# spacejam/loghisto

Hardware: NVIDIA H100
Metric: histogram ingest throughput (samples/s) (higher is better)
Workload: dtype f64

## Files before the change

### loghisto_b200/csrc/lh_api.cu

```cuda
#include "../../include/loghisto_b200.h"
#include "lh_kernels.cuh"

#include <algorithm>
#include <cmath>
#include <condition_variable>
#include <cstdio>
#include <cstring>
#include <mutex>
#include <new>
#include <string>
#include <thread>
#include <vector>
#include <unistd.h>

using namespace lh;

namespace {

struct WriterEvent { cudaStream_t stream; cudaEvent_t ev; };

struct Scope { uint64_t ticket; int buf; cudaStream_t stream; std::thread::id thread; };
static_assert(sizeof(Prec) == sizeof(((lh_recorder *)0)->prec) && offsetof(lh_recorder, prec) % alignof(Prec) == 0,
              "lh_recorder.prec must hold an lh::Prec");

// ... 113 lines not shown
    uint32_t H = 0, C = 0;
    Prec pc{};
    Buffer buf[2];
    int active = 0;
    bool frozen = false;
    bool freezing = false;
    bool nnz_valid = false;
    cudaStream_t ingest_stream = nullptr, snap_stream = nullptr, copy_stream = nullptr;
    double *d_decomp = nullptr;
    unsigned long long *d_dropped = nullptr;
    double *d_ps[3] = {nullptr, nullptr, nullptr};
    char *d_res[3] = {nullptr, nullptr, nullptr};
    char *h_res[3] = {nullptr, nullptr, nullptr};
    cudaEvent_t res_done[3] = {nullptr, nullptr, nullptr};
    uint32_t res_np[3] = {0, 0, 0};
    uint64_t res_ticket[2] = {0, 0};
    uint64_t next_ticket = 1;
    uint32_t *d_nnz = nullptr, *d_offsets = nullptr;
    short *d_x_keys = nullptr; unsigned long long *d_x_counts = nullptr; size_t x_cap = 0;
    uint32_t *h_offsets = nullptr;
    short *h_x_keys = nullptr; unsigned long long *h_x_counts = nullptr; size_t hx_cap = 0;
    unsigned long long *h_counter_deltas = nullptr;
    std::vector<Slot> slots;
    uint64_t slot_seq = 0;
    size_t staging_bytes = 0;
    unsigned long long last_margin[2] = {0, 0};
    int k1_variant = kDefaultK1Variant;
    int k1_grid_mult = 1;
    int k1_reserve_sms = 0;
    int keyed_blocks_per_sm = 8;
    uint32_t hot_replicas = 1;
    int keyed_mode = 0;
    int64_t kp_chunk = 256 << 20;
    uint32_t wc_pf_tiles = 1;
    uint32_t wc_flush_samples = 24576;
    int wc_spt = 6;
    unsigned short *d_kp_queues = nullptr;
    unsigned int *d_kp_cnt = nullptr;
    uint4 *d_kp_rare = nullptr;
    size_t kp_cap = 0;
    int kp_parts = 0;
    const char *keyed_kernel = "";
    uint32_t comm_rank = 0, comm_world = 0;
    unsigned long long *d_comm = nullptr;
    unsigned int *d_comm_aux = nullptr;
    PeerMap peers[kMaxRanks];
    unsigned long long *d_red_buckets = nullptr;
    uint32_t *d_red_flags = nullptr;
    unsigned long long *d_red_counters = nullptr;
    bool view_reduced = false;
    bool view_counters_reduced = false;
    uint64_t comm_seq = 0;
    bool comm_two_shot = false;
    static constexpr int kCommRing = 8;
    cudaEvent_t comm_t0[kCommRing] = {}, comm_t1[kCommRing] = {};
    uint64_t ctx_id = 0;
    std::mutex rs_mu;
    cudaStream_t rs_stream = nullptr;
    unsigned long long *d_rs_rows = nullptr;
    uint32_t *d_rs_flags = nullptr, *d_rs_nnz = nullptr;
    bool rs_dirty = false;
    K1Variant k1[kNumK1Variants];
    static constexpr int kTimingRing = 16;
    cudaEvent_t ev_t0s[kTimingRing] = {}, ev_t1s[kTimingRing] = {};
    cudaEvent_t ev_t0 = nullptr, ev_t1 = nullptr;
    uint64_t ingest_seq = 0;
    bool timing_valid = false;
// ... 97 lines not shown
    const size_t cells = (size_t)ctx->H * 2u * ctx->pc.win;
    int grid = (int)std::min<size_t>((cells + 255) / 256, (size_t)ctx->sm_count * 16);
    k_fold_hot<<<grid, 256, 0, s>>>(ctx->buf[b].d_hot, ctx->buf[b].d_buckets, ctx->buf[b].d_flags, cells, ctx->hot_replicas, ctx->pc.win);
    LH_CUDA(ctx, cudaGetLastError());
    ctx->stats.kernel_launches++;
    ctx->buf[b].hot_pending = 0;
    return LH_OK;
}

KeyedOut keyed_out(lh_ctx *ctx, int b) {
    KeyedOut o{};
    o.hot = ctx->buf[b].d_hot; o.buckets = ctx->buf[b].d_buckets; o.flags = ctx->buf[b].d_flags;
    o.dropped = ctx->d_dropped; o.H = ctx->H;
    return o;
}

uint32_t ks_passes(const lh_ctx *ctx) {
    const uint32_t per_max = std::max<uint32_t>(1, (uint32_t)(KS_SMEM_BYTES / ((size_t)ctx->pc.win * 4)));
    return (ctx->H + per_max - 1) / per_max;
}

constexpr uint32_t KS_MAX_PASSES = 4;
bool small_route(const lh_ctx *ctx) { return ks_passes(ctx) <= KS_MAX_PASSES && ctx->keyed_mode == 0; }

template <typename IdT, typename ValT>
void launch_keyed_scalar(lh_ctx *ctx, const KeyedOut &ko, const IdT *ids, const ValT *vals, size_t n, cudaStream_t s) {
    if (!n) return;
    constexpr int T = 256;
    k_ingest_keyed<IdT, ValT, T><<<grid_1d(ctx, n, T, 1, ctx->keyed_blocks_per_sm), T, 0, s>>>(ids, vals, n, ko, ctx->pc);
    ctx->stats.kernel_launches++;
}

constexpr size_t kSmemBudget = 227 * 1024;
template <typename IdT, typename ValT, int SPT>
lh_status launch_keyed_wc_spt(lh_ctx *ctx, int b, const IdT *ids, const ValT *vals, size_t n4x4, cudaStream_t s, bool *used, size_t *taken,
                              const IdT *ids2 = nullptr, const long long *vals2 = nullptr, size_t n2 = 0, size_t *taken2 = nullptr) {
    *used = false;
    *taken = 0;
    if (taken2) *taken2 = 0;
    const int P = std::min(ctx->sm_count - ctx->k1_reserve_sms, (int)WC_MAX_PARTS);
    if (P < 8 || n4x4 + n2 == 0) return LH_OK;
    const uint32_t ids_per = (ctx->H + P - 1) / P;
    using S = WcShape<SPT>;
    const size_t hist_bytes = (((size_t)ids_per * ctx->pc.win + 3) & ~(size_t)3) * 4;
    uint32_t row_cap = 0;
    size_t smem = 0;
    for (uint32_t cap_try : {256u, 192u, 128u}) {
        smem = hist_bytes + 2 * WC_MAX_PARTS * 4 + (size_t)(P + 1) * (cap_try + WC_ROW_EXTRA) * 2;
        if (smem <= kSmemBudget) { row_cap = cap_try; break; }
    }
    if (!row_cap || (size_t)ids_per * ctx->pc.win > 65535) return LH_OK;
    if (ctx->keyed_mode != 2 && n4x4 + n2 < ((size_t)1 << 22)) return LH_OK;
    n4x4 = n4x4 / S::TILE * S::TILE;
    n2 = n2 / S::TILE * S::TILE;
    if (n4x4 + n2 == 0) return LH_OK;
    const size_t slice_max = std::max<size_t>(1, ((size_t)ctx->kp_chunk + (size_t)P * S::TILE - 1) / ((size_t)P * S::TILE));
    const size_t tiles_all = n4x4 / S::TILE + n2 / S::TILE;
    const size_t nchunks = (tiles_all + slice_max * P - 1) / (slice_max * P);
    const size_t slice_tiles = std::max<size_t>(1, (tiles_all + nchunks * P - 1) / (nchunks * P));
    const size_t expect = slice_max * S::TILE / P;
    const size_t cap = ((expect * 5 / 4 + 3 * WC_LINE + WC_LINE - 1) / WC_LINE) * WC_LINE;
    if (!ctx->d_kp_queues || ctx->kp_cap != cap || ctx->kp_parts != P) {
        cudaFree(ctx->d_kp_queues); cudaFree(ctx->d_kp_cnt); cudaFree(ctx->d_kp_rare);
        ctx->d_kp_queues = nullptr; ctx->d_kp_cnt = nullptr; ctx->d_kp_rare = nullptr;
        LH_CUDA(ctx, cudaMalloc(&ctx->d_kp_rare, (size_t)P * WC_RARE_CAP * sizeof(uint4)));
        LH_CUDA(ctx, cudaMalloc(&ctx->d_kp_queues, (size_t)2 * P * P * cap * sizeof(unsigned short)));
        LH_CUDA(ctx, cudaMalloc(&ctx->d_kp_cnt, ((size_t)2 * P * P + 1) * sizeof(unsigned int)));
        ctx->kp_cap = cap; ctx->kp_parts = P;
    }
    const void *fn = (const void *)k_ingest_keyed_wc<IdT, ValT, SPT, false>;
    if constexpr (std::is_same<ValT, double>::value) {
        if (n2) fn = (const void *)k_ingest_keyed_wc<IdT, double, SPT, true>;
    }
    LH_CUDA(ctx, cudaFuncSetAttribute(fn, cudaFuncAttributeMaxDynamicSharedMemorySize, (int)smem));
    unsigned int *d_barrier = ctx->d_kp_cnt + (size_t)2 * P * P;
    LH_CUDA(ctx, cudaMemsetAsync(d_barrier, 0, sizeof(unsigned int), s));
    WcParams prm{};
    prm.ids = ids; prm.vals = vals; prm.n = n4x4; prm.ids_per = ids_per; prm.cap = (uint32_t)cap;
    prm.ids2 = ids2; prm.vals2 = vals2; prm.n2 = n2;
    prm.inv_p = (uint32_t)(((uint64_t)1 << 32) / (uint64_t)P) + 1u;
    const double room = (double)row_cap - 63.0;
    const double m_max = std::pow((-3.5 + std::sqrt(3.5 * 3.5 + 4.0 * room)) / 2.0, 2.0);
    const uint32_t flush_samples = std::min<uint32_t>(ctx->wc_flush_samples, (uint32_t)(m_max * P));
    prm.flush_tiles = std::max<uint32_t>(1u, flush_samples / S::TILE);
    prm.pf_tiles = ctx->wc_pf_tiles;
    prm.row_cap = row_cap;
    prm.row_stride = row_cap + WC_ROW_EXTRA;
    prm.slice_tiles = (uint32_t)slice_tiles; prm.queues = ctx->d_kp_queues; prm.q_cnt = ctx->d_kp_cnt;
    prm.barrier = d_barrier; prm.rare = ctx->d_kp_rare; prm.o = keyed_out(ctx, b);
    Prec pc = ctx->pc;
    void *args[] = {&prm, &pc};
    LH_CUDA(ctx, cudaLaunchCooperativeKernel(fn, dim3(P), dim3(S::THREADS), args, smem, s));
    ctx->stats.kernel_launches++;
    *used = true;
    *taken = n4x4;
    if (taken2) *taken2 = n2;
    return LH_OK;
}
template <typename IdT, typename ValT>
lh_status launch_keyed_wc(lh_ctx *ctx, int b, const IdT *ids, const ValT *vals, size_t n4x4, cudaStream_t s, bool *used, size_t *taken,
                          const IdT *ids2 = nullptr, const long long *vals2 = nullptr, size_t n2 = 0, size_t *taken2 = nullptr) {
#define LH_WC_SHAPE(code) case code: return launch_keyed_wc_spt<IdT, ValT, code>(ctx, b, ids, vals, n4x4, s, used, taken, ids2, vals2, n2, taken2);
    switch (ctx->wc_spt) {
        LH_WC_SHAPE(6) LH_WC_SHAPE(4) LH_WC_SHAPE(3)
        default: return launch_keyed_wc_spt<IdT, ValT, 8>(ctx, b, ids, vals, n4x4, s, used, taken, ids2, vals2, n2, taken2);
    }
#undef LH_WC_SHAPE
}

template <typename IdT, typename ValT>
lh_status launch_keyed(lh_ctx *ctx, int b, const IdT *d_ids, const ValT *d_vals, size_t n, cudaStream_t s) {
    constexpr int T = 256;
    const KeyedOut ko = keyed_out(ctx, b);
    size_t done = 0;
    while (done < n) {
        const unsigned long long kCap = 0xFFFFFFFFull;
        if (ctx->buf[b].hot_pending >= kCap - (1ull << 30)) { lh_status st = fold_hot(ctx, b, s); if (st != LH_OK) return st; }
        size_t m = (size_t)std::min<unsigned long long>(n - done, kCap - ctx->buf[b].hot_pending);
        const IdT *ids = d_ids + done;
        const ValT *vals = d_vals + done;
        size_t head = std::min<size_t>(m, ((32u - ((uintptr_t)vals & 31u)) & 31u) / 8u);
        bool vec_ok = (((uintptr_t)(ids + head)) & (4 * sizeof(IdT) - 1)) == 0;
        size_t n4 = vec_ok ? (m - head) / 4 : 0;
        size_t tail_off = head + n4 * 4;
        if (!vec_ok) { head = 0; tail_off = 0; }
        launch_keyed_scalar(ctx, ko, ids, vals, head, s);
// ... 1294 lines not shown
    LH_ENTER(ctx);
    LH_CUDA(ctx, cudaMemcpy(d_dst, h_src, bytes, cudaMemcpyHostToDevice));
    return LH_OK;
}
extern "C" lh_status lh_memcpy_d2h(lh_ctx *ctx, void *h_dst, const void *d_src, size_t bytes) {
    LH_ENTER(ctx);
    LH_CUDA(ctx, cudaMemcpy(h_dst, d_src, bytes, cudaMemcpyDeviceToHost));
    return LH_OK;
}

extern "C" lh_status lh_tune(lh_ctx *ctx, const char *key, int64_t value) {
    LH_ENTER(ctx);
    if (!key) return fail(ctx, LH_ERR_INVALID, "key is NULL");
    if (!strcmp(key, "k1")) {
        if (value < 0 || value >= kNumK1Variants) return fail(ctx, LH_ERR_RANGE, "unknown k1 variant");
        ctx->k1_variant = (int)value;
        return LH_OK;
    }
    if (!strcmp(key, "k1_grid_mult")) {
        if (value < 1 || value > 64) return fail(ctx, LH_ERR_RANGE, "k1_grid_mult out of range");
        ctx->k1_grid_mult = (int)value;
        return LH_OK;
    }
    if (!strcmp(key, "k1_reserve_sms")) {
        if (value < 0 || value >= ctx->sm_count) return fail(ctx, LH_ERR_RANGE, "k1_reserve_sms out of range");
        ctx->k1_reserve_sms = (int)value;
        return LH_OK;
    }
    if (!strcmp(key, "keyed_mode")) {
        if (value < 0 || value > 2) return fail(ctx, LH_ERR_RANGE, "keyed_mode is 0 (auto), 1 (L2 atomics) or 2 (owner-partitioned, write-combining)");
        ctx->keyed_mode = (int)value;
        return LH_OK;
    }
    if (!strcmp(key, "wc_pf")) {
        if (value < 0 || value > 8) return fail(ctx, LH_ERR_RANGE, "wc_pf is 0 ... 8 tiles");
        ctx->wc_pf_tiles = (uint32_t)value;
        return LH_OK;
    }
    if (!strcmp(key, "wc_flush")) {
        if (value < 4096 || value > 65536) return fail(ctx, LH_ERR_RANGE, "wc_flush is 4096 ... 65536 samples");
        ctx->wc_flush_samples = (uint32_t)value;
        return LH_OK;
    }
    if (!strcmp(key, "wc_spt")) {
        if (value != 4 && value != 6 && value != 3 && value != 8)
            return fail(ctx, LH_ERR_RANGE, "wc_spt is a shape code: 6 (896 threads x 4 samples), 4 (1024 x 4), 3 (768 x 4) or 8 (512 x 8)");
        ctx->wc_spt = (int)value;
        return LH_OK;
    }
    if (!strcmp(key, "kp_chunk")) {
        if (value < (1 << 16) || value > ((int64_t)1 << 28)) return fail(ctx, LH_ERR_RANGE, "kp_chunk out of range");
        ctx->kp_chunk = value;
        return LH_OK;
    }
    if (!strcmp(key, "keyed_blocks_per_sm")) {
        if (value < 1 || value > 32) return fail(ctx, LH_ERR_RANGE, "keyed_blocks_per_sm out of range");
        ctx->keyed_blocks_per_sm = (int)value;
        return LH_OK;
    }
    return fail(ctx, LH_ERR_INVALID, "unknown tuning key");
}

extern "C" int32_t lh_k1_variant_count(void) { return kNumK1Variants; }
extern "C" int32_t lh_k1_variant_current(lh_ctx *ctx) { return ctx ? ctx->k1_variant : -1; }
extern "C" const char *lh_k1_variant_name(lh_ctx *ctx, int32_t i) {
    if (!ctx || i < 0 || i >= kNumK1Variants) return "";
    return ctx->k1[i].name;
}

extern "C" uint64_t lh_ingest_seq(lh_ctx *ctx) {
    if (!ctx) return 0;
// ... 24 lines not shown
```

### loghisto_b200/csrc/lh_kernels.cuh

```cuda
#pragma once
#include "../../include/loghisto_b200.h"
#include <type_traits>
#include "lh_device.cuh"

namespace lh {

struct f64x4 { double a, b, c, d; };
__device__ __forceinline__ uint64_t policy_evict_first() {
    uint64_t p;
    asm("createpolicy.fractional.L2::evict_first.b64 %0, 1.0;" : "=l"(p));
    return p;
}
__device__ __forceinline__ void ldg_stream_u64x4(const void *p, unsigned long long (&r)[4]) {
    const uint64_t pol = policy_evict_first();
    asm volatile("ld.global.nc.L1::no_allocate.L2::cache_hint.v2.b64 {%0, %1}, [%2], %3;"
                 : "=l"(r[0]), "=l"(r[1]) : "l"(p), "l"(pol));
    asm volatile("ld.global.nc.L1::no_allocate.L2::cache_hint.v2.b64 {%0, %1}, [%2], %3;"
                 : "=l"(r[2]), "=l"(r[3]) : "l"((const char *)p + 16), "l"(pol));
}
__device__ __forceinline__ f64x4 ldg_stream_f64x4(const void *p) {
    unsigned long long u[4];
    ldg_stream_u64x4(p, u);
    f64x4 r;
    r.a = __longlong_as_double((long long)u[0]); r.b = __longlong_as_double((long long)u[1]);
// ... 415 lines not shown
        if (__any_sync(0xFFFFFFFFu, any)) {
#pragma unroll
            for (int i = 0; i < 4; i++) {
                if (!flag[i]) continue;
                ValT rv;
                memcpy(&rv, &cur[i], 8);
                keyed_one<ValT>(cur_id[i], rv, pc, o, o.hot, pol);
                off[i] = trash_off;
            }
        }
#pragma unroll
        for (int i = 0; i < 4; i++) atomicAdd(reinterpret_cast<uint32_t *>(reinterpret_cast<char *>(ks_hist) + off[i]), 1u);
#pragma unroll
        for (int i = 0; i < 4; i++) { cur[i] = nxt[i]; cur_id[i] = nxt_id[i]; }
    }
    __syncthreads();
    for (uint32_t i = threadIdx.x; i < words; i += KS_THREADS) {
        const uint32_t c = ks_hist[i];
        if (!c) continue;
        const uint32_t lid = i / row, slot = i - lid * row;
        atomicAdd(&o.hot[(size_t)(id_lo + lid) * (2u * pc.win) + slot], c);
    }
}

constexpr int WC_MAX_PARTS = 160;
constexpr int WC_LINE = 64;

template <int SPT> struct WcShape {
    static constexpr int THREADS = SPT == 4 ? 1024 : SPT == 6 ? 896 : SPT == 3 ? 768 : 512;
    static constexpr int PER = SPT == 8 ? 8 : 4;
    static constexpr int TILE = THREADS * PER;
};
constexpr int WC_ROW_EXTRA = WC_LINE + 8;

struct WcParams {
    const void *ids;
    const void *vals;
    size_t n;
    const void *ids2;
    const void *vals2;
    size_t n2;
    uint32_t ids_per;
    uint32_t cap;
    uint32_t slice_tiles;
    uint32_t inv_p;
    uint32_t flush_tiles;
    uint32_t pf_tiles;
    uint32_t row_cap;
    uint32_t row_stride;
    unsigned short *queues;
    unsigned int *q_cnt;
    unsigned int *barrier;
    uint4 *rare;
    KeyedOut o;
};
constexpr uint32_t WC_RARE_CAP = 8192;

__device__ __forceinline__ void grid_barrier(unsigned int *bar, unsigned int target) {
    __syncthreads();
    if (threadIdx.x == 0) {
        __threadfence();
        atomicAdd(bar, 1u);
        unsigned int v;
        do {
            asm volatile("ld.acquire.gpu.global.u32 %0, [%1];" : "=r"(v) : "l"(bar) : "memory");
        } while (v < target);
    }
    __syncthreads();
}

__device__ __forceinline__ void wc_spill(uint32_t rec, uint32_t owner, uint32_t P, const Prec &pc, const KeyedOut &o) {
    const uint32_t lid = rec / pc.win, slot = rec - lid * pc.win, id = lid * P + owner;
    add_bucket_global(o.buckets + (size_t)id * 65536u, o.flags + id, slot, 1ull, pc.win);
}

template <typename IdT, typename ValT, int SPT, bool PAIR = false>
__global__ void __launch_bounds__(WcShape<SPT>::THREADS, 1)
k_ingest_keyed_wc(WcParams prm, Prec pc) {
    static_assert(!PAIR || std::is_same<ValT, double>::value, "the int64 segment rides on the float64 instantiation");
    using S = WcShape<SPT>;
    constexpr int WC_THREADS = S::THREADS;
    constexpr int GROUPS = S::PER / 4;
    extern __shared__ __align__(16) unsigned char wc_smem[];
    const uint32_t P = gridDim.x, p = blockIdx.x, tid = threadIdx.x;
    unsigned int *s_hist = reinterpret_cast<unsigned int *>(wc_smem);
    const uint32_t hist_words = prm.ids_per * pc.win;
    unsigned int *s_fill = s_hist + ((hist_words + 3u) & ~3u);
    unsigned int *s_off = s_fill + WC_MAX_PARTS;
    unsigned short *s_buf = reinterpret_cast<unsigned short *>(s_off + WC_MAX_PARTS);
    uint32_t fill_addr = smem_u32(s_fill);
    const uint32_t hist_addr = smem_u32(s_hist);
    asm volatile("mov.b32 %0, %0;" : "+r"(fill_addr));
    const uint32_t buf_addr = fill_addr + 2u * WC_MAX_PARTS * 4u;
    unsigned int *s_rare = s_fill + (WC_MAX_PARTS - 1);
    uint4 *rareq = prm.rare + (size_t)p * WC_RARE_CAP;
    uint32_t negP = 0u - P;
    asm volatile("mov.b32 %0, %0;" : "+r"(negP));

    for (uint32_t i = tid; i < hist_words; i += WC_THREADS) s_hist[i] = 0;
    if (tid < WC_MAX_PARTS) { s_fill[tid] = 0; s_off[tid] = 0; }
    uint32_t one_bits;
    asm volatile("mov.b32 %0, 0x3F800000;" : "=r"(one_bits));
    __syncthreads();

    const size_t tiles_seg0 = prm.n / S::TILE;
    const size_t tiles_total = tiles_seg0 + (PAIR ? prm.n2 / S::TILE : 0);
    const size_t chunk_tiles = (size_t)prm.slice_tiles * P;
    const size_t nchunks = (tiles_total + chunk_tiles - 1) / chunk_tiles;
    const IdT *ids = reinterpret_cast<const IdT *>(prm.ids);
    const unsigned int cap = prm.cap;
    const uint32_t row_cap = prm.row_cap, row_stride = prm.row_stride;


    unsigned long long cur[GROUPS][4], nxt[GROUPS][4];
    IdPack<IdT> cur_id[GROUPS], nxt_id[GROUPS];
    uint32_t since_flush = 0;
    const char *vptr = nullptr;
    const IdT *iptr = nullptr;
    const size_t pf_v = (size_t)prm.pf_tiles * S::TILE * 8, pf_i = (size_t)prm.pf_tiles * S::TILE;
    auto load_tile = [&](const char *vp, const IdT *ip, unsigned long long (&raw)[GROUPS][4], IdPack<IdT> (&idp)[GROUPS]) {
#pragma unroll
        for (int g = 0; g < GROUPS; g++) {
            load_vals4(vp, (size_t)g * WC_THREADS, raw[g]);
            idp[g].load(ip, (size_t)g * WC_THREADS);
        }
    };

    for (size_t c = 0; c < nchunks; c++) {
        const size_t par = c & 1;
        unsigned short *qset = prm.queues + par * (size_t)P * P * cap;
        unsigned int *cset = prm.q_cnt + par * (size_t)P * P;
        const bool last_chunk = c + 1 == nchunks;
        const size_t tile0 = c * chunk_tiles + (size_t)p * prm.slice_tiles;
        const uint32_t ntile_all = tile0 >= tiles_total ? 0u : (uint32_t)min((size_t)prm.slice_tiles, tiles_total - tile0);
        auto bin_tile = [&](unsigned long long (&raw)[GROUPS][4], IdPack<IdT> (&idp)[GROUPS], const bool as_i64) {
            if constexpr (PAIR) {
                if (as_i64) {
#pragma unroll
                    for (int g = 0; g < GROUPS; g++)
#pragma unroll
                        for (int j = 0; j < 4; j++) raw[g][j] = (unsigned long long)__double_as_longlong(__ll2double_rn((long long)raw[g][j]));
                }
            }
#pragma unroll
            for (int g = 0; g < GROUPS; g++) {
                double v[4];
#pragma unroll
                for (int j = 0; j < 4; j++) { ValT r; memcpy(&r, &raw[g][j], 8); v[j] = sample_to_f64<ValT>(r); }
                uint32_t idx[4];
                bool flag[4];
                bucket_offsets_v2<4, false, 0>(v, pc, one_bits, idx, flag);
                bool any = false;
#pragma unroll
                for (int j = 0; j < 4; j++) {
                    const uint32_t id = idp[g].get(j);
                    const uint32_t lid = __umulhi(id, prm.inv_p), owner = lid * negP + id;
                    const uint32_t rec = lid * pc.win + idx[j];
                    const bool rare = flag[j] | (id >= prm.o.H);
                    const uint32_t oe = rare ? P : owner;
                    uint32_t pos;
                    asm volatile("atom.shared.add.u32 %0, [%1], 1;" : "=r"(pos) : "r"(fill_addr + oe * 4u) : "memory");
                    flag[j] = rare | (pos >= row_cap);
                    if (!flag[j])
                        asm volatile("st.shared.u16 [%0], %1;" ::"r"(buf_addr + (oe * row_stride + pos) * 2u), "h"((unsigned short)rec) : "memory");
                    any |= flag[j];
                }
                if (__any_sync(0xFFFFFFFFu, any)) {
#pragma unroll
                    for (int j = 0; j < 4; j++)
                        if (flag[j]) {
                            const unsigned int at = atomicAdd(s_rare, 1u);
                            if (at < WC_RARE_CAP) rareq[at] = make_uint4((unsigned int)raw[g][j], (unsigned int)(raw[g][j] >> 32), idp[g].get(j), 0u);
                            else keyed_one_slow<ValT>(idp[g].get(j), raw[g][j], pc, prm.o);
                        }
                }
            }
            if (++since_flush == prm.flush_tiles) {
                since_flush = 0;
                __syncthreads();
                constexpr uint32_t GROUPS_PER_WARP = 8;
                const uint32_t sub = (tid & 31) >> 2, k4 = (tid & 3) * 2;
                for (uint32_t base = (tid >> 5) * GROUPS_PER_WARP; base < P; base += (WC_THREADS / 32) * GROUPS_PER_WARP) {
                    const uint32_t o = base + sub;
                    const bool act = o < P;
                    unsigned int n = 0, nfull = 0, off0 = 0;
                    uint4 keep0 = make_uint4(0, 0, 0, 0), keep1 = keep0;
                    uint4 *src = reinterpret_cast<uint4 *>(s_buf + (act ? o : 0) * row_stride);
                    if (act) {
                        n = min(s_fill[o], row_cap);
                        nfull = n / WC_LINE;
                        off0 = s_off[o];
                        unsigned short *qbase = qset + ((size_t)o * P + p) * cap;
                        keep0 = src[nfull * 8 + k4];
                        keep1 = src[nfull * 8 + k4 + 1];
                        for (unsigned int l = 0; l < nfull; l++) {
                            if (off0 + WC_LINE <= cap) {
                                uint4 *dst = reinterpret_cast<uint4 *>(qbase + off0);
                                const uint4 a0 = src[l * 8 + k4], a1 = src[l * 8 + k4 + 1];
                                dst[k4] = a0;
                                dst[k4 + 1] = a1;
                                off0 += WC_LINE;
                            } else if (k4 == 0) {
                                const unsigned short *r = s_buf + o * row_stride + l * WC_LINE;
                                for (unsigned int k = 0; k < (unsigned int)WC_LINE; k++) wc_spill(r[k], o, P, pc, prm.o);
                            }
                        }
                    }
                    __syncwarp();
                    if (act) {
                        if (nfull) { src[k4] = keep0; src[k4 + 1] = keep1; }
                        if (k4 == 0) { s_off[o] = off0; s_fill[o] = n - nfull * WC_LINE; }
                    }
                }
                __syncthreads();
            }
        };
        for (int part = 0; part < (PAIR ? 2 : 1); part++) {
            const size_t lo = part == 0 ? tile0 : max(tile0, tiles_seg0);
            const size_t hi = part == 0 ? min(tile0 + ntile_all, tiles_seg0) : tile0 + ntile_all;
            if (hi <= lo) continue;
            const uint32_t ntile = (uint32_t)(hi - lo);
            const bool as_i64 = part == 1;
            const size_t first = (part == 0 ? lo : lo - tiles_seg0) * S::TILE + (size_t)tid * 4;
            vptr = reinterpret_cast<const char *>(part == 0 ? prm.vals : prm.vals2) + first * 8;
            iptr = (part == 0 ? ids : reinterpret_cast<const IdT *>(prm.ids2)) + first;
            load_tile(vptr, iptr, cur, cur_id);
            auto prefetch_ahead = [&](uint32_t tile_loaded) {
                if (prm.pf_tiles && tile_loaded + prm.pf_tiles < ntile) {
#pragma unroll
                    for (int g = 0; g < GROUPS; g++) {
                        asm volatile("prefetch.global.L2 [%0];" ::"l"(vptr + pf_v + (size_t)g * WC_THREADS * 32));
                        if ((tid & 3) == 0) asm volatile("prefetch.global.L2 [%0];" ::"l"(iptr + pf_i + (size_t)g * WC_THREADS * 4));
                    }
                }
            };
            for (uint32_t t = 0; t < ntile; t += 2) {
                vptr += (size_t)S::TILE * 8;
                iptr += S::TILE;
                if (t + 1 < ntile) load_tile(vptr, iptr, nxt, nxt_id);
                prefetch_ahead(t + 1);
                bin_tile(cur, cur_id, as_i64);
                if (t + 1 >= ntile) break;
                vptr += (size_t)S::TILE * 8;
                iptr += S::TILE;
                if (t + 2 < ntile) load_tile(vptr, iptr, cur, cur_id);
                prefetch_ahead(t + 2);
                bin_tile(nxt, nxt_id, as_i64);
            }
        }
        __syncthreads();
        {
            const unsigned int nr = min(*s_rare, WC_RARE_CAP);
            for (unsigned int i = tid; i < nr; i += WC_THREADS) {
                const uint4 e = rareq[i];
                ValT r;
                const unsigned long long raw = ((unsigned long long)e.y << 32) | e.x;
                memcpy(&r, &raw, 8);
                keyed_one_direct<ValT>(e.z, r, pc, prm.o);
            }
            __syncthreads();
            if (tid == 0) *s_rare = 0;
        }
        if (last_chunk) {
            if (tid < P) {
                const uint32_t o = tid;
                const unsigned int n = min(s_fill[o], row_cap);
                unsigned int off0 = s_off[o];
                const uint4 *src = reinterpret_cast<const uint4 *>(s_buf + o * row_stride);
                for (unsigned int l = 0; l * WC_LINE < n; l++) {
                    const unsigned int nrec = min((unsigned int)WC_LINE, n - l * WC_LINE);
                    if (off0 + WC_LINE <= cap) {
                        uint4 *dst = reinterpret_cast<uint4 *>(qset + ((size_t)o * P + p) * cap + off0);
#pragma unroll
                        for (int k = 0; k < 8; k++) dst[k] = src[l * 8 + k];
                        off0 += nrec;
                    } else {
                        const unsigned short *r = s_buf + o * row_stride + l * WC_LINE;
                        for (unsigned int k = 0; k < nrec; k++) wc_spill(r[k], o, P, pc, prm.o);
                    }
                }
                s_off[o] = off0;
                s_fill[o] = 0;
            }
            __syncthreads();
        }
        if (tid < P) { cset[(size_t)tid * P + p] = s_off[tid]; }
        grid_barrier(prm.barrier, (unsigned int)((c + 1) * (size_t)P));
        if (tid < P) s_off[tid] = __ldcg(&cset[(size_t)p * P + tid]);
        __syncthreads();
        {
            const unsigned short *qmine = qset + (size_t)p * P * cap;
            const uint32_t lane = tid & 31;
#define LH_WC_INC2(word)                                                                                              \
            asm volatile("red.shared.add.u32 [%0], 1;" ::"r"(hist_addr + (((word) << 2) & 0x3FFFCu)) : "memory");     \
            asm volatile("red.shared.add.u32 [%0], 1;" ::"r"(hist_addr + (((word) >> 14) & 0x3FFFCu)) : "memory");
            for (uint32_t w = tid >> 5; w < P; w += WC_THREADS / 32) {
                const unsigned int cnt = s_off[w];
                const unsigned short *q = qmine + (size_t)w * cap;
                const uint4 *qv = reinterpret_cast<const uint4 *>(q);
                const unsigned int nv = cnt >> 3;
#pragma unroll 2
                for (unsigned int i = lane; i < nv; i += 32) {
                    const uint4 v4 = __ldcg(qv + i);
                    LH_WC_INC2(v4.x) LH_WC_INC2(v4.y) LH_WC_INC2(v4.z) LH_WC_INC2(v4.w)
                }
                const unsigned int r0 = nv * 8u + lane;
                if (r0 < cnt) asm volatile("red.shared.add.u32 [%0], 1;" ::"r"(hist_addr + (unsigned int)__ldcg(q + r0) * 4u) : "memory");
            }
#undef LH_WC_INC2
        }
        __syncthreads();
        if (tid < P) s_off[tid] = 0;
    }
    __syncthreads();
    for (uint32_t lid = 0; lid < prm.ids_per; lid++) {
        const uint32_t id = lid * P + p;
        if (id >= prm.o.H) break;
        int any = 0;
        for (uint32_t slot = tid; slot < pc.win; slot += WC_THREADS) {
            const unsigned int cnt = s_hist[lid * pc.win + slot];
            if (cnt) { atomicAdd(&prm.o.buckets[(size_t)id * 65536u + slot], (unsigned long long)cnt); any = 1; }
        }
        any = __syncthreads_or(any);
        if (any && tid == 0) mark(&prm.o.flags[id], 1u);
    }
}

__global__ void k_fold_hot(unsigned int *__restrict__ hot, unsigned long long *__restrict__ buckets, uint32_t *__restrict__ flags,
                           size_t cells, uint32_t replicas, uint32_t win) {
    const size_t stride = (size_t)gridDim.x * blockDim.x;
    const uint32_t row = 2u * win;
    for (size_t i = (size_t)blockIdx.x * blockDim.x + threadIdx.x; i < cells; i += stride) {
        unsigned long long sum = 0;
        for (uint32_t r = 0; r < replicas; r++) {
            unsigned int *cell = hot + (size_t)r * cells + i;
            if (*cell) sum += atomicExch(cell, 0u);
        }
        if (sum) {
            size_t h = i / row;
            uint32_t slot = (uint32_t)(i - h * row);
            atomicAdd(&buckets[h * 65536u + slot_to_key16(slot, win)], sum);
            mark(&flags[h], 1u);
        }
    }
}

constexpr int K2_SMEM_COUNTERS = 8192;

template <typename IdT, int THREADS>
__global__ void __launch_bounds__(THREADS)
k_counter_add_smem(const IdT *__restrict__ ids, const unsigned long long *__restrict__ amounts, size_t n,
                   unsigned long long *__restrict__ counters, uint32_t C,
// ... 706 lines not shown
```

Measured before the change: 399.1 billion.

## Split cooperative keyed binning kernel into per-chunk bin and drain kernels with TMA ring

Replaces the single cooperative persistent kernel, which used a software grid barrier and double-buffered queues, with two kernels launched per chunk: a binning kernel and a drain kernel. The binning kernel loads input tiles through an mbarrier-synchronised bulk-copy ring in shared memory instead of register double-buffering plus L2 prefetch. It also no longer holds the per-partition histogram, which frees shared memory for more ring stages. The drain kernel builds the histogram with 1024 threads. This drops the grid barrier and the wc_pf knob, at the cost of two launches per chunk and rebuilding the shared-memory histogram per chunk.

New measurement: 399.1 billion, median of 6. Within noise of the previous version (+0.0%).

```diff
diff --git a/loghisto_b200/csrc/lh_api.cu b/loghisto_b200/csrc/lh_api.cu
--- a/loghisto_b200/csrc/lh_api.cu
+++ b/loghisto_b200/csrc/lh_api.cu
@@ -169,7 +169,6 @@
     uint32_t hot_replicas = 1;
     int keyed_mode = 0;
     int64_t kp_chunk = 256 << 20;
-    uint32_t wc_pf_tiles = 1;
     uint32_t wc_flush_samples = 24576;
     int wc_spt = 6;
     unsigned short *d_kp_queues = nullptr;
@@ -333,6 +332,8 @@
 }
 
 constexpr size_t kSmemBudget = 227 * 1024;
+static_assert(wc_bin_fixed_smem(WC_MAX_PARTS, 256) + 2 * WcRing<4096, 4>::STAGE_BYTES <= kSmemBudget,
+              "the binning kernel's input ring must hold two of the largest tiles (4096 samples, u32 ids) at any P");
 template <typename IdT, typename ValT, int SPT>
 lh_status launch_keyed_wc_spt(lh_ctx *ctx, int b, const IdT *ids, const ValT *vals, size_t n4x4, cudaStream_t s, bool *used, size_t *taken,
                               const IdT *ids2 = nullptr, const long long *vals2 = nullptr, size_t n2 = 0, size_t *taken2 = nullptr) {
@@ -365,17 +366,21 @@
         cudaFree(ctx->d_kp_queues); cudaFree(ctx->d_kp_cnt); cudaFree(ctx->d_kp_rare);
         ctx->d_kp_queues = nullptr; ctx->d_kp_cnt = nullptr; ctx->d_kp_rare = nullptr;
         LH_CUDA(ctx, cudaMalloc(&ctx->d_kp_rare, (size_t)P * WC_RARE_CAP * sizeof(uint4)));
-        LH_CUDA(ctx, cudaMalloc(&ctx->d_kp_queues, (size_t)2 * P * P * cap * sizeof(unsigned short)));
-        LH_CUDA(ctx, cudaMalloc(&ctx->d_kp_cnt, ((size_t)2 * P * P + 1) * sizeof(unsigned int)));
+        LH_CUDA(ctx, cudaMalloc(&ctx->d_kp_queues, (size_t)P * P * cap * sizeof(unsigned short)));
+        LH_CUDA(ctx, cudaMalloc(&ctx->d_kp_cnt, (size_t)P * P * sizeof(unsigned int)));
         ctx->kp_cap = cap; ctx->kp_parts = P;
     }
-    const void *fn = (const void *)k_ingest_keyed_wc<IdT, ValT, SPT, false>;
+    const size_t stage_bytes = WcRing<S::TILE, sizeof(IdT)>::STAGE_BYTES;
+    const size_t bin_fixed = wc_bin_fixed_smem(P, row_cap);
+    const uint32_t stages = (uint32_t)std::min<size_t>(WC_MAX_STAGES, (kSmemBudget - bin_fixed) / stage_bytes);
+    const size_t smem_bin = bin_fixed + stages * stage_bytes;
+    const size_t smem_drain = hist_bytes + WC_MAX_PARTS * 4;
+    void (*bin)(WcParams, Prec, uint32_t) = k_keyed_wc_bin<IdT, ValT, SPT, false>;
     if constexpr (std::is_same<ValT, double>::value) {
-        if (n2) fn = (const void *)k_ingest_keyed_wc<IdT, double, SPT, true>;
-    }
-    LH_CUDA(ctx, cudaFuncSetAttribute(fn, cudaFuncAttributeMaxDynamicSharedMemorySize, (int)smem));
-    unsigned int *d_barrier = ctx->d_kp_cnt + (size_t)2 * P * P;
-    LH_CUDA(ctx, cudaMemsetAsync(d_barrier, 0, sizeof(unsigned int), s));
+        if (n2) bin = k_keyed_wc_bin<IdT, double, SPT, true>;
+    }
+    LH_CUDA(ctx, cudaFuncSetAttribute((const void *)bin, cudaFuncAttributeMaxDynamicSharedMemorySize, (int)smem_bin));
+    LH_CUDA(ctx, cudaFuncSetAttribute((const void *)k_keyed_wc_drain, cudaFuncAttributeMaxDynamicSharedMemorySize, (int)smem_drain));
     WcParams prm{};
     prm.ids = ids; prm.vals = vals; prm.n = n4x4; prm.ids_per = ids_per; prm.cap = (uint32_t)cap;
     prm.ids2 = ids2; prm.vals2 = vals2; prm.n2 = n2;
@@ -384,15 +389,16 @@
     const double m_max = std::pow((-3.5 + std::sqrt(3.5 * 3.5 + 4.0 * room)) / 2.0, 2.0);
     const uint32_t flush_samples = std::min<uint32_t>(ctx->wc_flush_samples, (uint32_t)(m_max * P));
     prm.flush_tiles = std::max<uint32_t>(1u, flush_samples / S::TILE);
-    prm.pf_tiles = ctx->wc_pf_tiles;
     prm.row_cap = row_cap;
     prm.row_stride = row_cap + WC_ROW_EXTRA;
+    prm.stages = stages; prm.stage_bytes = (uint32_t)stage_bytes;
     prm.slice_tiles = (uint32_t)slice_tiles; prm.queues = ctx->d_kp_queues; prm.q_cnt = ctx->d_kp_cnt;
-    prm.barrier = d_barrier; prm.rare = ctx->d_kp_rare; prm.o = keyed_out(ctx, b);
-    Prec pc = ctx->pc;
-    void *args[] = {&prm, &pc};
-    LH_CUDA(ctx, cudaLaunchCooperativeKernel(fn, dim3(P), dim3(S::THREADS), args, smem, s));
-    ctx->stats.kernel_launches++;
+    prm.rare = ctx->d_kp_rare; prm.o = keyed_out(ctx, b);
+    for (size_t c = 0; c < nchunks; c++) {
+        bin<<<P, S::THREADS, smem_bin, s>>>(prm, ctx->pc, (uint32_t)c);
+        k_keyed_wc_drain<<<P, WC_DRAIN_THREADS, smem_drain, s>>>(prm, ctx->pc);
+        ctx->stats.kernel_launches += 2;
+    }
     *used = true;
     *taken = n4x4;
     if (taken2) *taken2 = n2;
@@ -1753,11 +1759,6 @@
         ctx->keyed_mode = (int)value;
         return LH_OK;
     }
-    if (!strcmp(key, "wc_pf")) {
-        if (value < 0 || value > 8) return fail(ctx, LH_ERR_RANGE, "wc_pf is 0 ... 8 tiles");
-        ctx->wc_pf_tiles = (uint32_t)value;
-        return LH_OK;
-    }
     if (!strcmp(key, "wc_flush")) {
         if (value < 4096 || value > 65536) return fail(ctx, LH_ERR_RANGE, "wc_flush is 4096 ... 65536 samples");
         ctx->wc_flush_samples = (uint32_t)value;
diff --git a/loghisto_b200/csrc/lh_kernels.cuh b/loghisto_b200/csrc/lh_kernels.cuh
--- a/loghisto_b200/csrc/lh_kernels.cuh
+++ b/loghisto_b200/csrc/lh_kernels.cuh
@@ -471,6 +471,8 @@
     static constexpr int TILE = THREADS * PER;
 };
 constexpr int WC_ROW_EXTRA = WC_LINE + 8;
+constexpr uint32_t WC_MAX_STAGES = 4;
+constexpr int WC_DRAIN_THREADS = 1024;
 
 struct WcParams {
     const void *ids;
@@ -484,28 +486,20 @@
     uint32_t slice_tiles;
     uint32_t inv_p;
     uint32_t flush_tiles;
-    uint32_t pf_tiles;
     uint32_t row_cap;
     uint32_t row_stride;
+    uint32_t stages;
+    uint32_t stage_bytes;
     unsigned short *queues;
     unsigned int *q_cnt;
-    unsigned int *barrier;
     uint4 *rare;
     KeyedOut o;
 };
 constexpr uint32_t WC_RARE_CAP = 8192;
 
-__device__ __forceinline__ void grid_barrier(unsigned int *bar, unsigned int target) {
-    __syncthreads();
-    if (threadIdx.x == 0) {
-        __threadfence();
-        atomicAdd(bar, 1u);
-        unsigned int v;
-        do {
-            asm volatile("ld.acquire.gpu.global.u32 %0, [%1];" : "=r"(v) : "l"(bar) : "memory");
-        } while (v < target);
-    }
-    __syncthreads();
+template <int TILE, int ID_BYTES> struct WcRing { static constexpr uint32_t STAGE_BYTES = TILE * (8 + ID_BYTES) + 16; };
+constexpr size_t wc_bin_fixed_smem(uint32_t P, uint32_t row_cap) {
+    return 2 * WC_MAX_STAGES * 8 + 2 * WC_MAX_PARTS * 4 + (size_t)(P + 1) * (row_cap + WC_ROW_EXTRA) * 2;
 }
 
 __device__ __forceinline__ void wc_spill(uint32_t rec, uint32_t owner, uint32_t P, const Prec &pc, const KeyedOut &o) {
@@ -515,248 +509,252 @@
 
 template <typename IdT, typename ValT, int SPT, bool PAIR = false>
 __global__ void __launch_bounds__(WcShape<SPT>::THREADS, 1)
-k_ingest_keyed_wc(WcParams prm, Prec pc) {
+k_keyed_wc_bin(WcParams prm, Prec pc, uint32_t chunk) {
     static_assert(!PAIR || std::is_same<ValT, double>::value, "the int64 segment rides on the float64 instantiation");
     using S = WcShape<SPT>;
     constexpr int WC_THREADS = S::THREADS;
     constexpr int GROUPS = S::PER / 4;
-    extern __shared__ __align__(16) unsigned char wc_smem[];
+    constexpr uint32_t VAL_BYTES = S::TILE * 8;
+    extern __shared__ __align__(128) unsigned char wc_smem[];
     const uint32_t P = gridDim.x, p = blockIdx.x, tid = threadIdx.x;
-    unsigned int *s_hist = reinterpret_cast<unsigned int *>(wc_smem);
-    const uint32_t hist_words = prm.ids_per * pc.win;
-    unsigned int *s_fill = s_hist + ((hist_words + 3u) & ~3u);
+    const uint32_t stages = prm.stages, stage_bytes = prm.stage_bytes;
+    uint64_t *full = reinterpret_cast<uint64_t *>(wc_smem + (size_t)stages * stage_bytes);
+    uint64_t *empty = full + WC_MAX_STAGES;
+    unsigned int *s_fill = reinterpret_cast<unsigned int *>(empty + WC_MAX_STAGES);
     unsigned int *s_off = s_fill + WC_MAX_PARTS;
     unsigned short *s_buf = reinterpret_cast<unsigned short *>(s_off + WC_MAX_PARTS);
     uint32_t fill_addr = smem_u32(s_fill);
-    const uint32_t hist_addr = smem_u32(s_hist);
     asm volatile("mov.b32 %0, %0;" : "+r"(fill_addr));
     const uint32_t buf_addr = fill_addr + 2u * WC_MAX_PARTS * 4u;
+    const uint32_t ring_addr = smem_u32(wc_smem);
     unsigned int *s_rare = s_fill + (WC_MAX_PARTS - 1);
     uint4 *rareq = prm.rare + (size_t)p * WC_RARE_CAP;
     uint32_t negP = 0u - P;
     asm volatile("mov.b32 %0, %0;" : "+r"(negP));
 
-    for (uint32_t i = tid; i < hist_words; i += WC_THREADS) s_hist[i] = 0;
     if (tid < WC_MAX_PARTS) { s_fill[tid] = 0; s_off[tid] = 0; }
+    if (tid == 0) {
+        for (uint32_t s = 0; s < stages; s++) { mbar_init(&full[s], 1); mbar_init(&empty[s], WC_THREADS / 32); }
+        asm volatile("fence.mbarrier_init.release.cluster;" ::: "memory");
+    }
     uint32_t one_bits;
     asm volatile("mov.b32 %0, 0x3F800000;" : "=r"(one_bits));
     __syncthreads();
 
     const size_t tiles_seg0 = prm.n / S::TILE;
     const size_t tiles_total = tiles_seg0 + (PAIR ? prm.n2 / S::TILE : 0);
-    const size_t chunk_tiles = (size_t)prm.slice_tiles * P;
-    const size_t nchunks = (tiles_total + chunk_tiles - 1) / chunk_tiles;
-    const IdT *ids = reinterpret_cast<const IdT *>(prm.ids);
+    const size_t tile0 = ((size_t)chunk * P + p) * prm.slice_tiles;
+    const uint32_t ntile = tile0 >= tiles_total ? 0u : (uint32_t)min((size_t)prm.slice_tiles, tiles_total - tile0);
+    const uint32_t skew0 = (uint32_t)(uintptr_t)prm.ids & 15u, skew1 = (uint32_t)(uintptr_t)prm.ids2 & 15u;
     const unsigned int cap = prm.cap;
     const uint32_t row_cap = prm.row_cap, row_stride = prm.row_stride;
 
-
-    unsigned long long cur[GROUPS][4], nxt[GROUPS][4];
-    IdPack<IdT> cur_id[GROUPS], nxt_id[GROUPS];
-    uint32_t since_flush = 0;
-    const char *vptr = nullptr;
-    const IdT *iptr = nullptr;
-    const size_t pf_v = (size_t)prm.pf_tiles * S::TILE * 8, pf_i = (size_t)prm.pf_tiles * S::TILE;
-    auto load_tile = [&](const char *vp, const IdT *ip, unsigned long long (&raw)[GROUPS][4], IdPack<IdT> (&idp)[GROUPS]) {
+    auto issue = [&](uint32_t u, uint32_t s) {
+        const uint64_t pol = policy_evict_first();
+        const size_t t = tile0 + u;
+        const bool seg1 = PAIR && t >= tiles_seg0;
+        const size_t first = (seg1 ? t - tiles_seg0 : t) * S::TILE;
+        const uint32_t skew = seg1 ? skew1 : skew0;
+        const char *v = reinterpret_cast<const char *>(seg1 ? prm.vals2 : prm.vals) + first * 8;
+        const char *i = reinterpret_cast<const char *>(seg1 ? prm.ids2 : prm.ids) + first * sizeof(IdT) - skew;
+        const uint32_t ibytes = (skew + S::TILE * (uint32_t)sizeof(IdT) + 15u) & ~15u;
+        unsigned char *st = wc_smem + (size_t)s * stage_bytes;
+        mbar_expect_tx(&full[s], VAL_BYTES + ibytes);
+        bulk_g2s(st, v, VAL_BYTES, &full[s], pol);
+        bulk_g2s(st + VAL_BYTES, i, ibytes, &full[s], pol);
+    };
+    if (tid == 0)
+        for (uint32_t u = 0; u < min(stages, ntile); u++) issue(u, u);
+
+    uint32_t slot = 0, phase = 0, since_flush = 0;
+    for (uint32_t u = 0; u < ntile; u++) {
+        const bool as_i64 = PAIR && tile0 + u >= tiles_seg0;
+        const uint32_t skew = as_i64 ? skew1 : skew0;
+        unsigned long long raw[GROUPS][4];
+        uint32_t idv[GROUPS][4];
+        mbar_wait(&full[slot], phase);
+        {
+            const uint32_t st = ring_addr + slot * stage_bytes;
+#pragma unroll
+            for (int g = 0; g < GROUPS; g++)
+#pragma unroll
+                for (int h = 0; h < 2; h++) {
+                    const uint32_t q = (uint32_t)(g * 2 + h) * WC_THREADS + tid;
+                    asm volatile("ld.shared.v2.u64 {%0, %1}, [%2];" : "=l"(raw[g][2 * h]), "=l"(raw[g][2 * h + 1]) : "r"(st + q * 16u) : "memory");
+                    if constexpr (sizeof(IdT) == 2) {
+                        uint32_t w;
+                        asm volatile("ld.shared.u32 %0, [%1];" : "=r"(w) : "r"(st + VAL_BYTES + skew + q * 4u) : "memory");
+                        idv[g][2 * h] = w & 0xFFFFu;
+                        idv[g][2 * h + 1] = w >> 16;
+                    } else {
+                        asm volatile("ld.shared.v2.u32 {%0, %1}, [%2];" : "=r"(idv[g][2 * h]), "=r"(idv[g][2 * h + 1])
+                                     : "r"(st + VAL_BYTES + skew + q * 8u) : "memory");
+                    }
+                }
+        }
+        asm volatile("fence.proxy.async.shared::cta;" ::: "memory");
+        __syncwarp();
+        if ((tid & 31) == 0) mbar_arrive(&empty[slot]);
+        if (tid < 32 && u > 0 && u - 1 + stages < ntile) {
+            const uint32_t ps = slot == 0 ? stages - 1 : slot - 1;
+            const uint32_t pp = slot == 0 ? phase ^ 1u : phase;
+            mbar_wait(&empty[ps], pp);
+            if (tid == 0) issue(u - 1 + stages, ps);
+            __syncwarp();
+        }
+        if (++slot == stages) { slot = 0; phase ^= 1u; }
+
+        if constexpr (PAIR) {
+            if (as_i64) {
+#pragma unroll
+                for (int g = 0; g < GROUPS; g++)
+#pragma unroll
+                    for (int j = 0; j < 4; j++) raw[g][j] = (unsigned long long)__double_as_longlong(__ll2double_rn((long long)raw[g][j]));
+            }
+        }
 #pragma unroll
         for (int g = 0; g < GROUPS; g++) {
-            load_vals4(vp, (size_t)g * WC_THREADS, raw[g]);
-            idp[g].load(ip, (size_t)g * WC_THREADS);
-        }
-    };
-
-    for (size_t c = 0; c < nchunks; c++) {
-        const size_t par = c & 1;
-        unsigned short *qset = prm.queues + par * (size_t)P * P * cap;
-        unsigned int *cset = prm.q_cnt + par * (size_t)P * P;
-        const bool last_chunk = c + 1 == nchunks;
-        const size_t tile0 = c * chunk_tiles + (size_t)p * prm.slice_tiles;
-        const uint32_t ntile_all = tile0 >= tiles_total ? 0u : (uint32_t)min((size_t)prm.slice_tiles, tiles_total - tile0);
-        auto bin_tile = [&](unsigned long long (&raw)[GROUPS][4], IdPack<IdT> (&idp)[GROUPS], const bool as_i64) {
-            if constexpr (PAIR) {
-                if (as_i64) {
-#pragma unroll
-                    for (int g = 0; g < GROUPS; g++)
-#pragma unroll
-                        for (int j = 0; j < 4; j++) raw[g][j] = (unsigned long long)__double_as_longlong(__ll2double_rn((long long)raw[g][j]));
-                }
-            }
-#pragma unroll
-            for (int g = 0; g < GROUPS; g++) {
-                double v[4];
-#pragma unroll
-                for (int j = 0; j < 4; j++) { ValT r; memcpy(&r, &raw[g][j], 8); v[j] = sample_to_f64<ValT>(r); }
-                uint32_t idx[4];
-                bool flag[4];
-                bucket_offsets_v2<4, false, 0>(v, pc, one_bits, idx, flag);
-                bool any = false;
-#pragma unroll
-                for (int j = 0; j < 4; j++) {
-                    const uint32_t id = idp[g].get(j);
-                    const uint32_t lid = __umulhi(id, prm.inv_p), owner = lid * negP + id;
-                    const uint32_t rec = lid * pc.win + idx[j];
-                    const bool rare = flag[j] | (id >= prm.o.H);
-                    const uint32_t oe = rare ? P : owner;
-                    uint32_t pos;
-                    asm volatile("atom.shared.add.u32 %0, [%1], 1;" : "=r"(pos) : "r"(fill_addr + oe * 4u) : "memory");
-                    flag[j] = rare | (pos >= row_cap);
-                    if (!flag[j])
-                        asm volatile("st.shared.u16 [%0], %1;" ::"r"(buf_addr + (oe * row_stride + pos) * 2u), "h"((unsigned short)rec) : "memory");
-                    any |= flag[j];
-                }
-                if (__any_sync(0xFFFFFFFFu, any)) {
-#pragma unroll
-                    for (int j = 0; j < 4; j++)
-                        if (flag[j]) {
-                            const unsigned int at = atomicAdd(s_rare, 1u);
-                            if (at < WC_RARE_CAP) rareq[at] = make_uint4((unsigned int)raw[g][j], (unsigned int)(raw[g][j] >> 32), idp[g].get(j), 0u);
-                            else keyed_one_slow<ValT>(idp[g].get(j), raw[g][j], pc, prm.o);
-                        }
-                }
-            }
-            if (++since_flush == prm.flush_tiles) {
-                since_flush = 0;
-                __syncthreads();
-                constexpr uint32_t GROUPS_PER_WARP = 8;
-                const uint32_t sub = (tid & 31) >> 2, k4 = (tid & 3) * 2;
-                for (uint32_t base = (tid >> 5) * GROUPS_PER_WARP; base < P; base += (WC_THREADS / 32) * GROUPS_PER_WARP) {
-                    const uint32_t o = base + sub;
-                    const bool act = o < P;
-                    unsigned int n = 0, nfull = 0, off0 = 0;
-                    uint4 keep0 = make_uint4(0, 0, 0, 0), keep1 = keep0;
-                    uint4 *src = reinterpret_cast<uint4 *>(s_buf + (act ? o : 0) * row_stride);
-                    if (act) {
-                        n = min(s_fill[o], row_cap);
-                        nfull = n / WC_LINE;
-                        off0 = s_off[o];
-                        unsigned short *qbase = qset + ((size_t)o * P + p) * cap;
-                        keep0 = src[nfull * 8 + k4];
-                        keep1 = src[nfull * 8 + k4 + 1];
-                        for (unsigned int l = 0; l < nfull; l++) {
-                            if (off0 + WC_LINE <= cap) {
-                                uint4 *dst = reinterpret_cast<uint4 *>(qbase + off0);
-                                const uint4 a0 = src[l * 8 + k4], a1 = src[l * 8 + k4 + 1];
-                                dst[k4] = a0;
-                                dst[k4 + 1] = a1;
-                                off0 += WC_LINE;
-                            } else if (k4 == 0) {
-                                const unsigned short *r = s_buf + o * row_stride + l * WC_LINE;
-                                for (unsigned int k = 0; k < (unsigned int)WC_LINE; k++) wc_spill(r[k], o, P, pc, prm.o);
-                            }
+            double v[4];
+#pragma unroll
+            for (int j = 0; j < 4; j++) { ValT r; memcpy(&r, &raw[g][j], 8); v[j] = sample_to_f64<ValT>(r); }
+            uint32_t idx[4];
+            bool flag[4];
+            bucket_offsets_v2<4, false, 0>(v, pc, one_bits, idx, flag);
+            bool any = false;
+#pragma unroll
+            for (int j = 0; j < 4; j++) {
+                const uint32_t id = idv[g][j];
+                const uint32_t lid = __umulhi(id, prm.inv_p), owner = lid * negP + id;
+                const uint32_t rec = lid * pc.win + idx[j];
+                const bool rare = flag[j] | (id >= prm.o.H);
+                const uint32_t oe = rare ? P : owner;
+                uint32_t pos;
+                asm volatile("atom.shared.add.u32 %0, [%1], 1;" : "=r"(pos) : "r"(fill_addr + oe * 4u) : "memory");
+                flag[j] = rare | (pos >= row_cap);
+                if (!flag[j])
+                    asm volatile("st.shared.u16 [%0], %1;" ::"r"(buf_addr + (oe * row_stride + pos) * 2u), "h"((unsigned short)rec) : "memory");
+                any |= flag[j];
+            }
+            if (__any_sync(0xFFFFFFFFu, any)) {
+#pragma unroll
+                for (int j = 0; j < 4; j++)
+                    if (flag[j]) {
+                        const unsigned int at = atomicAdd(s_rare, 1u);
+                        if (at < WC_RARE_CAP) rareq[at] = make_uint4((unsigned int)raw[g][j], (unsigned int)(raw[g][j] >> 32), idv[g][j], 0u);
+                        else keyed_one_slow<ValT>(idv[g][j], raw[g][j], pc, prm.o);
+                    }
+            }
+        }
+        if (++since_flush == prm.flush_tiles) {
+            since_flush = 0;
+            __syncthreads();
+            constexpr uint32_t GROUPS_PER_WARP = 8;
+            const uint32_t sub = (tid & 31) >> 2, k4 = (tid & 3) * 2;
+            for (uint32_t base = (tid >> 5) * GROUPS_PER_WARP; base < P; base += (WC_THREADS / 32) * GROUPS_PER_WARP) {
+                const uint32_t o = base + sub;
+                const bool act = o < P;
+                unsigned int n = 0, nfull = 0, off0 = 0;
+                uint4 keep0 = make_uint4(0, 0, 0, 0), keep1 = keep0;
+                uint4 *src = reinterpret_cast<uint4 *>(s_buf + (act ? o : 0) * row_stride);
+                if (act) {
+                    n = min(s_fill[o], row_cap);
+                    nfull = n / WC_LINE;
+                    off0 = s_off[o];
+                    unsigned short *qbase = prm.queues + ((size_t)o * P + p) * cap;
+                    keep0 = src[nfull * 8 + k4];
+                    keep1 = src[nfull * 8 + k4 + 1];
+                    for (unsigned int l = 0; l < nfull; l++) {
+                        if (off0 + WC_LINE <= cap) {
+                            uint4 *dst = reinterpret_cast<uint4 *>(qbase + off0);
+                            const uint4 a0 = src[l * 8 + k4], a1 = src[l * 8 + k4 + 1];
+                            dst[k4] = a0;
+                            dst[k4 + 1] = a1;
+                            off0 += WC_LINE;
+                        } else if (k4 == 0) {
+                            const unsigned short *r = s_buf + o * row_stride + l * WC_LINE;
+                            for (unsigned int k = 0; k < (unsigned int)WC_LINE; k++) wc_spill(r[k], o, P, pc, prm.o);
                         }
                     }
-                    __syncwarp();
-                    if (act) {
-                        if (nfull) { src[k4] = keep0; src[k4 + 1] = keep1; }
-                        if (k4 == 0) { s_off[o] = off0; s_fill[o] = n - nfull * WC_LINE; }
-                    }
                 }
-                __syncthreads();
-            }
-        };
-        for (int part = 0; part < (PAIR ? 2 : 1); part++) {
-            const size_t lo = part == 0 ? tile0 : max(tile0, tiles_seg0);
-            const size_t hi = part == 0 ? min(tile0 + ntile_all, tiles_seg0) : tile0 + ntile_all;
-            if (hi <= lo) continue;
-            const uint32_t ntile = (uint32_t)(hi - lo);
-            const bool as_i64 = part == 1;
-            const size_t first = (part == 0 ? lo : lo - tiles_seg0) * S::TILE + (size_t)tid * 4;
-            vptr = reinterpret_cast<const char *>(part == 0 ? prm.vals : prm.vals2) + first * 8;
-            iptr = (part == 0 ? ids : reinterpret_cast<const IdT *>(prm.ids2)) + first;
-            load_tile(vptr, iptr, cur, cur_id);
-            auto prefetch_ahead = [&](uint32_t tile_loaded) {
-                if (prm.pf_tiles && tile_loaded + prm.pf_tiles < ntile) {
-#pragma unroll
-                    for (int g = 0; g < GROUPS; g++) {
-                        asm volatile("prefetch.global.L2 [%0];" ::"l"(vptr + pf_v + (size_t)g * WC_THREADS * 32));
-                        if ((tid & 3) == 0) asm volatile("prefetch.global.L2 [%0];" ::"l"(iptr + pf_i + (size_t)g * WC_THREADS * 4));
-                    }
+                __syncwarp();
+                if (act) {
+                    if (nfull) { src[k4] = keep0; src[k4 + 1] = keep1; }
+                    if (k4 == 0) { s_off[o] = off0; s_fill[o] = n - nfull * WC_LINE; }
                 }
-            };
-            for (uint32_t t = 0; t < ntile; t += 2) {
-                vptr += (size_t)S::TILE * 8;
-                iptr += S::TILE;
-                if (t + 1 < ntile) load_tile(vptr, iptr, nxt, nxt_id);
-                prefetch_ahead(t + 1);
-                bin_tile(cur, cur_id, as_i64);
-                if (t + 1 >= ntile) break;
-                vptr += (size_t)S::TILE * 8;
-                iptr += S::TILE;
-                if (t + 2 < ntile) load_tile(vptr, iptr, cur, cur_id);
-                prefetch_ahead(t + 2);
-                bin_tile(nxt, nxt_id, as_i64);
-            }
-        }
-        __syncthreads();
-        {
-            const unsigned int nr = min(*s_rare, WC_RARE_CAP);
-            for (unsigned int i = tid; i < nr; i += WC_THREADS) {
-                const uint4 e = rareq[i];
-                ValT r;
-                const unsigned long long raw = ((unsigned long long)e.y << 32) | e.x;
-                memcpy(&r, &raw, 8);
-                keyed_one_direct<ValT>(e.z, r, pc, prm.o);
             }
             __syncthreads();
-            if (tid == 0) *s_rare = 0;
-        }
-        if (last_chunk) {
-            if (tid < P) {
-                const uint32_t o = tid;
-                const unsigned int n = min(s_fill[o], row_cap);
-                unsigned int off0 = s_off[o];
-                const uint4 *src = reinterpret_cast<const uint4 *>(s_buf + o * row_stride);
-                for (unsigned int l = 0; l * WC_LINE < n; l++) {
-                    const unsigned int nrec = min((unsigned int)WC_LINE, n - l * WC_LINE);
-                    if (off0 + WC_LINE <= cap) {
-                        uint4 *dst = reinterpret_cast<uint4 *>(qset + ((size_t)o * P + p) * cap + off0);
-#pragma unroll
-                        for (int k = 0; k < 8; k++) dst[k] = src[l * 8 + k];
-                        off0 += nrec;
-                    } else {
-                        const unsigned short *r = s_buf + o * row_stride + l * WC_LINE;
-                        for (unsigned int k = 0; k < nrec; k++) wc_spill(r[k], o, P, pc, prm.o);
-                    }
-                }
-                s_off[o] = off0;
-                s_fill[o] = 0;
-            }
-            __syncthreads();
-        }
-        if (tid < P) { cset[(size_t)tid * P + p] = s_off[tid]; }
-        grid_barrier(prm.barrier, (unsigned int)((c + 1) * (size_t)P));
-        if (tid < P) s_off[tid] = __ldcg(&cset[(size_t)p * P + tid]);
-        __syncthreads();
-        {
-            const unsigned short *qmine = qset + (size_t)p * P * cap;
-            const uint32_t lane = tid & 31;
+        }
+    }
+    __syncthreads();
+    {
+        const unsigned int nr = min(*s_rare, WC_RARE_CAP);
+        for (unsigned int i = tid; i < nr; i += WC_THREADS) {
+            const uint4 e = rareq[i];
+            ValT r;
+            const unsigned long long raw = ((unsigned long long)e.y << 32) | e.x;
+            memcpy(&r, &raw, 8);
+            keyed_one_direct<ValT>(e.z, r, pc, prm.o);
+        }
+    }
+    if (tid < P) {
+        const uint32_t o = tid;
+        const unsigned int n = min(s_fill[o], row_cap);
+        unsigned int off0 = s_off[o];
+        const uint4 *src = reinterpret_cast<const uint4 *>(s_buf + o * row_stride);
+        for (unsigned int l = 0; l * WC_LINE < n; l++) {
+            const unsigned int nrec = min((unsigned int)WC_LINE, n - l * WC_LINE);
+            if (off0 + WC_LINE <= cap) {
+                uint4 *dst = reinterpret_cast<uint4 *>(prm.queues + ((size_t)o * P + p) * cap + off0);
+#pragma unroll
+                for (int k = 0; k < 8; k++) dst[k] = src[l * 8 + k];
+                off0 += nrec;
+            } else {
+                const unsigned short *r = s_buf + o * row_stride + l * WC_LINE;
+                for (unsigned int k = 0; k < nrec; k++) wc_spill(r[k], o, P, pc, prm.o);
+            }
+        }
+        prm.q_cnt[(size_t)o * P + p] = off0;
+    }
+}
+
+__global__ void __launch_bounds__(WC_DRAIN_THREADS, 1)
+k_keyed_wc_drain(WcParams prm, Prec pc) {
+    extern __shared__ __align__(16) unsigned int wd_smem[];
+    const uint32_t P = gridDim.x, p = blockIdx.x, tid = threadIdx.x;
+    unsigned int *s_hist = wd_smem;
+    const uint32_t hist_words = prm.ids_per * pc.win;
+    unsigned int *s_cnt = s_hist + ((hist_words + 3u) & ~3u);
+    const uint32_t hist_addr = smem_u32(s_hist);
+    for (uint32_t i = tid; i < hist_words; i += WC_DRAIN_THREADS) s_hist[i] = 0;
+    if (tid < P) s_cnt[tid] = __ldcg(&prm.q_cnt[(size_t)p * P + tid]);
+    __syncthreads();
+    {
+        const unsigned short *qmine = prm.queues + (size_t)p * P * prm.cap;
+        const uint32_t lane = tid & 31;
 #define LH_WC_INC2(word)                                                                                              \
-            asm volatile("red.shared.add.u32 [%0], 1;" ::"r"(hist_addr + (((word) << 2) & 0x3FFFCu)) : "memory");     \
-            asm volatile("red.shared.add.u32 [%0], 1;" ::"r"(hist_addr + (((word) >> 14) & 0x3FFFCu)) : "memory");
-            for (uint32_t w = tid >> 5; w < P; w += WC_THREADS / 32) {
-                const unsigned int cnt = s_off[w];
-                const unsigned short *q = qmine + (size_t)w * cap;
-                const uint4 *qv = reinterpret_cast<const uint4 *>(q);
-                const unsigned int nv = cnt >> 3;
+        asm volatile("red.shared.add.u32 [%0], 1;" ::"r"(hist_addr + (((word) << 2) & 0x3FFFCu)) : "memory");         \
+        asm volatile("red.shared.add.u32 [%0], 1;" ::"r"(hist_addr + (((word) >> 14) & 0x3FFFCu)) : "memory");
+        for (uint32_t w = tid >> 5; w < P; w += WC_DRAIN_THREADS / 32) {
+            const unsigned int cnt = s_cnt[w];
+            const unsigned short *q = qmine + (size_t)w * prm.cap;
+            const uint4 *qv = reinterpret_cast<const uint4 *>(q);
+            const unsigned int nv = cnt >> 3;
 #pragma unroll 2
-                for (unsigned int i = lane; i < nv; i += 32) {
-                    const uint4 v4 = __ldcg(qv + i);
-                    LH_WC_INC2(v4.x) LH_WC_INC2(v4.y) LH_WC_INC2(v4.z) LH_WC_INC2(v4.w)
-                }
-                const unsigned int r0 = nv * 8u + lane;
-                if (r0 < cnt) asm volatile("red.shared.add.u32 [%0], 1;" ::"r"(hist_addr + (unsigned int)__ldcg(q + r0) * 4u) : "memory");
-            }
+            for (unsigned int i = lane; i < nv; i += 32) {
+                const uint4 v4 = __ldcg(qv + i);
+                LH_WC_INC2(v4.x) LH_WC_INC2(v4.y) LH_WC_INC2(v4.z) LH_WC_INC2(v4.w)
+            }
+            const unsigned int r0 = nv * 8u + lane;
+            if (r0 < cnt) asm volatile("red.shared.add.u32 [%0], 1;" ::"r"(hist_addr + (unsigned int)__ldcg(q + r0) * 4u) : "memory");
+        }
 #undef LH_WC_INC2
-        }
-        __syncthreads();
-        if (tid < P) s_off[tid] = 0;
     }
     __syncthreads();
     for (uint32_t lid = 0; lid < prm.ids_per; lid++) {
         const uint32_t id = lid * P + p;
         if (id >= prm.o.H) break;
         int any = 0;
-        for (uint32_t slot = tid; slot < pc.win; slot += WC_THREADS) {
+        for (uint32_t slot = tid; slot < pc.win; slot += WC_DRAIN_THREADS) {
             const unsigned int cnt = s_hist[lid * pc.win + slot];
             if (cnt) { atomicAdd(&prm.o.buckets[(size_t)id * 65536u + slot], (unsigned long long)cnt); any = 1; }
         }
```
